# JuliaReinforcementLearning/ReinforcementLearning.jl

Hardware: AMD Instinct MI355X
Metric: env_steps_per_sec (higher is better)
Workload: dtype f32; 1 GPU; ppo_cartpole_4096env_per_gpu (BASELINE.json configs[3] per GPU); n_envs_per_gpu=4096, rollout_T=32, actor=4->256->2 relu, critic=4->256->1 relu, n_params=3331, n_epochs=4, n_microbatches=4, microbatch=32768, parallelism=single GPU

## Files before the change

### __graft_entry__.py

```python
import os
import sys

ROOT = os.path.dirname(os.path.abspath(__file__))
PKG = os.path.join(ROOT, "reinforcementlearning.jl_amd")
for p in (ROOT, PKG):
    if p not in sys.path:
        sys.path.insert(0, p)


def build():
    import importlib.util

    spec = importlib.util.spec_from_file_location("rlhip_build", os.path.join(PKG, "build.py"))
    mod = importlib.util.module_from_spec(spec)
    spec.loader.exec_module(mod)
    so = mod.build()
    assert os.path.exists(so)
    assert os.path.exists(mod.build(variant="bounds"))
    import oracle

    oracle.build()
    import rlhip

    missing = [s for s in rlhip._lib.declared_symbols() if not hasattr(rlhip._lib.lib, s)]
    assert not missing, f"librlhip.so does not export: {missing}"
    build_abi_host()
    build_micro_checks()


MICRO_CHECKS = ("mfma_f32_l1", "mfma_f32_4x4", "tanh_sel", "mfma_valu_overlap", "wave_simd_map", "log_sampling", "trig_f32arg")
MICRO_FLAGS = {"mfma_valu_overlap": ["-fno-slp-vectorize", "-fno-vectorize"], "trig_f32arg": ["-pthread"]}


def build_micro_checks():
    import subprocess

    outs = []
    for name in MICRO_CHECKS:
        src = os.path.join(ROOT, "tools", "micro", name + ".hip")
        out = os.path.join(ROOT, "tools", "micro", name + ".bin")
        if os.path.exists(out) and os.path.getmtime(out) >= max(
                [os.path.getmtime(src)] + [os.path.getmtime(os.path.join(PKG, "csrc", f)) for f in os.listdir(os.path.join(PKG, "csrc"))
                                           if f.endswith(".h")]):
            outs.append(out)
            continue
        cmd = ["/opt/rocm/bin/hipcc", "--offload-arch=gfx950", "-O3", "-std=c++17", "-ffp-contract=off", "-Wno-unused-result", "-Wno-unused-value",
               "-I" + os.path.join(ROOT, "include")] + MICRO_FLAGS.get(name, []) + [src, "-o", out]
        r = subprocess.run(cmd, capture_output=True, text=True)
        if r.returncode != 0:
            raise RuntimeError(f"hipcc failed for {src}:\n{r.stdout}\n{r.stderr}")
        outs.append(out)
    return outs


def build_abi_host():
    import subprocess

    src = os.path.join(ROOT, "tests", "abi_host", "abi_host.c")
    out = os.path.join(ROOT, "tests", "abi_host", "abi_host.bin")
    cmd = ["gcc", "-std=c99", "-O2", "-Wall", "-I" + os.path.join(ROOT, "include"), src, "-o", out,
           "-L" + os.path.join(PKG, "lib"), "-lrlhip", "-Wl,-rpath,$ORIGIN/../../reinforcementlearning.jl_amd/lib",
           "-Wl,-rpath,/opt/rocm/lib", "-lm"]
    r = subprocess.run(cmd, capture_output=True, text=True)
    if r.returncode != 0:
        raise RuntimeError(f"gcc failed for abi_host.c:\n{r.stdout}\n{r.stderr}")
    return out


def smoke():
    import numpy as np
    import torch

    import oracle
    import rlhip

    assert torch.cuda.is_available(), "smoke() needs an MI355X"
    torch.cuda.set_device(0)
    n, T = 256, 8
    env = rlhip.HipVecEnv("cartpole", n, seed=7)
    pol = rlhip.PPOPolicy(env, update_freq=T, n_epochs=1, n_microbatches=2)
    p0 = pol.params.cpu().numpy().copy()
    pol.rollout_()
    pol.gae_()
    tr = pol.trajectory
    oenv = oracle.VecEnv("cartpole", n, seed=7)
    ocfg = oracle.ppo_default(n_epochs=1, n_microbatches=2)
    otr = oracle.PPOTraj(0, n, T)
    oracle.ppo_rollout(oenv, T, ocfg, p0, otr, 0)
    agree = (tr.action_i.cpu().numpy() == otr.action_i).mean()
    assert agree > 0.995, f"sampled actions agree only {agree:.4f}"
    if agree == 1.0:
        assert np.array_equal(tr.terminal.cpu().numpy(), otr.terminal)
        np.testing.assert_allclose(tr.obs.cpu().numpy(), otr.obs, rtol=1e-5, atol=1e-6)
        np.testing.assert_allclose(tr.value.cpu().numpy(), otr.value, rtol=1e-5, atol=1e-6)
    o = oracle.generalized_advantage_estimation(tr.reward.cpu().numpy().T, tr.value.cpu().numpy().T, 0.99, 0.95,
                                                terminal=tr.terminal.cpu().numpy().T, dims=2, dtype=np.float32)
    assert np.array_equal(tr.adv.cpu().numpy(), o.T)
    pol.grad_(0, 0)
    total, bm = n * T, (n * T) // 2
    perm = np.array([oracle.permute(pol.seed, 0, total, b) for b in range(bm)])
    t, i = perm // n, perm % n
    obs = tr.obs.cpu().numpy()[t, :, i].T.copy()
    flat = lambda x: x.cpu().numpy().reshape(-1)[perm]
    g, losses = oracle.ppo_loss_grad(ocfg, 4, 2, p0, obs, flat(tr.action_i), flat(tr.logp), flat(tr.adv), flat(tr.ret))
    gerr = np.abs(pol.grad.cpu().numpy() - g).max() / np.abs(g).max()
    assert gerr <= 1e-6, f"gradient differs from the oracle by {gerr:.2e} of max|g| (bar 1e-6; measured 8e-8)"
    np.testing.assert_allclose(pol.losses.cpu().numpy(), losses, rtol=1e-4, atol=1e-6)
    pol.update_()
    torch.cuda.synchronize()
    assert torch.isfinite(pol.params).all() and not torch.equal(pol.params.cpu(), torch.tensor(p0))
    print(f"smoke ok: {n} envs x {T} steps, loss {float(pol.losses[0]):.5f}, actions agree {agree:.4f}")
    smoke_bench_shape(np, torch, oracle, rlhip)


def smoke_bench_shape(np, torch, oracle, rlhip):
    n, T = 4096, 32
    oracle.use_all_cores(True)
    try:
        env = rlhip.HipVecEnv("cartpole", n, seed=123)
        pol = rlhip.PPOPolicy(env, update_freq=T, hidden=256, seed=123)
        p0 = pol.params.cpu().numpy().copy()
        pol.rollout_()
        tr = pol.trajectory
        oenv = oracle.VecEnv("cartpole", n, seed=123)
        ocfg = oracle.ppo_default(hidden=256)
        otr = oracle.PPOTraj(0, n, T)
        oracle.ppo_rollout(oenv, T, ocfg, p0, otr, 0)
        ga = tr.action_i.cpu().numpy()
        flipped = (ga != otr.action_i).any(0)
        assert flipped.sum() <= 8, f"{flipped.sum()} of {n} envs took another action than the oracle's"
        keep = ~flipped
        assert np.array_equal(tr.terminal.cpu().numpy()[:, keep], otr.terminal[:, keep])
        np.testing.assert_allclose(tr.obs.cpu().numpy()[:, :, keep], otr.obs[:, :, keep], rtol=1e-5, atol=1e-6)
        np.testing.assert_allclose(tr.value.cpu().numpy()[:, keep], otr.value[:, keep], rtol=1e-5, atol=1e-6)
        mb, total = 1, n * T
        bm = total // pol.cfg.n_microbatches
        pol.grad_(0, mb)
        perm = np.array([oracle.permute(pol.seed, 0, total, mb * bm + b) for b in range(bm)])
        t, i = perm // n, perm % n
        flat = lambda x: x.cpu().numpy().reshape(-1)[perm]
        g, losses = oracle.ppo_loss_grad(ocfg, 4, 2, p0, tr.obs.cpu().numpy()[t, :, i].T.copy(), flat(tr.action_i), flat(tr.logp),
                                         flat(tr.adv), flat(tr.ret))
        gerr = np.abs(pol.grad.cpu().numpy() - g).max() / np.abs(g).max()
        assert bm == 32768 and gerr <= 1e-6, f"32768-sample gradient differs from the oracle by {gerr:.2e} of max|g| (bar 1e-6)"
        np.testing.assert_allclose(pol.losses.cpu().numpy(), losses, rtol=1e-4, atol=1e-6)
        print(f"smoke ok at the bench shape: {n} envs x {T} steps ({int(flipped.sum())} envs flipped an action), micro-batch of "
              f"{bm}: gradient within {gerr:.1e} of max|g|")
    finally:
        oracle.use_all_cores(False)


if __name__ == "__main__":
    build()
    if len(sys.argv) > 1 and sys.argv[1] == "smoke":
        smoke()
```

### reinforcementlearning.jl_amd/csrc/ppo.hip

```cpp
#include "env_device.h"
#include "mlp_device.h"
#include "select_device.h"
#include "select_decide.h"
#include "ppo_common.h"
#include "ppo_sample_device.h"

extern "C" int32_t rlhip_clip_adam_f32(float* params, float* grad, float* m, float* v, float* beta_pow,
                                       int64_t n, float grad_scale, float clip_norm, float lr, float beta1,
                                       float beta2, float eps, float* gn_out, rlhip_stream_t stream);
extern "C" int32_t rlhip_gae_returns_f32(float* advantages, float* returns, const float* rewards,
                                         const float* values, const uint8_t* terminal, int64_t n_env,
                                         int64_t T, float gamma, float lambda, rlhip_stream_t stream);

namespace rlhip {

__global__ void counters_advance_kernel(uint32_t* ctr, uint32_t d0, uint32_t d1) {
    ctr[0] += d0;
    ctr[1] += d1;
}

#ifdef RLHIP_ROLLOUT_TIMING
__device__ unsigned int g_rollout_exact_waves = 0;
#define RT_COUNT_EXACT()                                                   \
    do {                                                                   \
        if ((threadIdx.x & 63) == 0) atomicAdd(&g_rollout_exact_waves, 1u); \
    } while (0)
#define RT_PRINT_EXACT()                                                                                              \
    do {                                                                                                              \
        if (blockIdx.x == 0 && threadIdx.x == 0)                                                                      \
            printf("exact-selection wavefronts so far: %u\n", atomicAdd(&g_rollout_exact_waves, 0u));                  \
    } while (0)
#define RT_DECL long long rt_[8] = {0, 0, 0, 0, 0, 0, 0, 0}, rt_last_ = 0
#define RT_START() rt_last_ = (long long)__builtin_amdgcn_s_memtime()
#define RT_STAMP(k)                                                   \
    do {                                                              \
        __builtin_amdgcn_sched_barrier(0);                            \
        const long long now_ = (long long)__builtin_amdgcn_s_memtime(); \
        rt_[k] += now_ - rt_last_;                                    \
        rt_last_ = now_;                                              \
        __builtin_amdgcn_sched_barrier(0);                            \
    } while (0)
#define RT_PRINT(tag)                                                                                             \
    do {                                                                                                          \
        if (blockIdx.x == 0 && (threadIdx.x & 255) == 0)                                                          \
            printf("%s T=%d: %lld %lld %lld %lld %lld %lld %lld %lld\n", tag, T, rt_[0], rt_[1], rt_[2], rt_[3], rt_[4], \
                   rt_[5], rt_[6], rt_[7]);                                                                       \
    } while (0)
#else
#define RT_COUNT_EXACT()
#define RT_PRINT_EXACT()
#define RT_DECL
#define RT_START()
#define RT_STAMP(k)
#define RT_PRINT(tag)
#endif

template <class P, int H, int L, int ACT, int NOA, int HEAD>
__global__ __launch_bounds__(512, 1) void rollout_split_kernel(P p, EnvArrays<float> st, int64_t n, int T,
                                                               PolicyDesc pd, const float* __restrict__ params,
                                                               uint64_t seed, uint32_t env_id_base,
                                                               uint32_t vec_step0_in, const uint32_t* __restrict__ ctr, TrajPtrs tr,
                                                               int store_state, float select_margin) {
    const uint32_t vec_step0 = vec_step0_in + (ctr ? ctr[0] : 0u);
    constexpr int NS = P::ODIM;
    constexpr int HPL = H / L;
    constexpr int EPB = 256 / L;
    constexpr int NOISE_CH = 16;
    const int cont = HEAD == 0 ? pd.cont : (HEAD == 1 ? 1 : 0);
    const int na = HEAD == 0 ? pd.na : (HEAD == 1 ? 1 : HEAD);
    if (HEAD != 0) p.continuous = cont;
    const int role = (int)(threadIdx.x >> 8);
    const int tl = (int)(threadIdx.x & 255);
    int64_t gl = (int64_t)blockIdx.x * 256 + tl;
    int64_t env = gl / L;
    const int sub = (int)(gl % L);
    const int eg = tl / L;
    const bool active = env < n;
    if (!active) env = n - 1;
    const bool writer = active && sub == 0;
    const uint32_t id = env_id_base + (uint32_t)env;

    __shared__ double l_noise[2][EPB][NOISE_CH][MAXO];
    __shared__ float4 l_step[2][EPB][2];
    __shared__ float2 l_lse[HEAD == 2 ? EPB : 1][NOISE_CH];

    if (role == 0) {
        __builtin_amdgcn_s_setprio(3);
        NetRegs<NS, HPL> A;
        load_net<NS, HPL>(A, params, H, pd.nout_a, sub, L);
        LaneState<float> e;
#pragma unroll
        for (int k = 0; k < P::SDIM; ++k) e.s[k] = st.s[k][env];
        e.t = st.t[env];
        e.episode = st.episode[env];
        float last_r = 0.0f;
        bool last_d = false;
        [[maybe_unused]] const double sel_km = decide2_slope((double)select_margin);
        RT_DECL;
        __syncthreads();
        RT_START();
        for (int t = 0; t < T; ++t) {
            double nz[MAXO];
#pragma unroll
            for (int k = 0; k < MAXO; ++k)
                nz[k] = (HEAD == 2 ? k >= 2 : k < na) ? l_noise[(t / NOISE_CH) & 1][eg][t & (NOISE_CH - 1)][k] : 0.0;
            float x[4] = {0.f, 0.f, 0.f, 0.f};
            env_obs1(p, e, x);
            RT_STAMP(0);
            float oa[MAXO];
            net_forward<NS, HPL, L, ACT, NOA>(A, x, oa);
            RT_STAMP(1);
            int32_t ai;
            float af, lp;
            float sel_d = 0.0f;
            if constexpr (HEAD == 2) {
                float sel_e;
                bool decided;
                ai = decide2_logits(oa[0], oa[1], nz[2], nz[3], sel_km, &sel_e, &decided);
                decide2_operands(oa[0], oa[1], sel_e, ai, &lp, &sel_d);
                if (__builtin_amdgcn_ballot_w64(!decided) != 0) {
                    RT_COUNT_EXACT();
                    const double nzx[MAXO] = {l_noise[(t / NOISE_CH) & 1][eg][t & (NOISE_CH - 1)][0],
                                              l_noise[(t / NOISE_CH) & 1][eg][t & (NOISE_CH - 1)][1], 0.0, 0.0};
                    float lp_exact, xa0, xa1;
                    const int32_t ax = categorical_select1(RegLogits{oa}, NoMask{}, na, NoiseRegs{nzx}, &lp_exact);
                    if (!decided) ai = ax;
                    select2_operands(oa[0], oa[1], &xa0, &xa1, &sel_d);
                    lp = ai ? xa1 : xa0;
                }
                af = 0.0f;
            } else {
                policy_select(cont, na, oa, nz, ai, af, lp);
            }
            RT_STAMP(2);
            env_step1(p, e, ai, af, last_r, last_d);
            if (last_d) env_reset1(p, e, seed, id);
            RT_STAMP(3);
            if (sub == 0) {
                l_step[t & 1][eg][0] = make_float4(x[0], x[1], x[2], x[3]);
                if constexpr (HEAD == 2)
                    l_step[t & 1][eg][1] = make_float4(lp, sel_d, __int_as_float(ai | (last_d ? 0x100 : 0)), last_r);
                else
                    l_step[t & 1][eg][1] = make_float4(lp, cont ? af : __int_as_float(ai), last_r, last_d ? 1.0f : 0.0f);
            }
            RT_STAMP(4);
            __syncthreads();
            RT_STAMP(5);
        }
        RT_PRINT("actor wave: obs/noise | forward | select | env step | record | barrier");
        if (HEAD == 2) RT_PRINT_EXACT();
        {
            float x[4] = {0.f, 0.f, 0.f, 0.f};
            env_obs1(p, e, x);
            if (sub == 0) l_step[T & 1][eg][0] = make_float4(x[0], x[1], x[2], x[3]);
            __syncthreads();
        }
        if (writer && store_state) {
#pragma unroll
            for (int k = 0; k < P::SDIM; ++k) st.s[k][env] = e.s[k];
            st.t[env] = e.t;
            st.episode[env] = e.episode;
            if (T > 0) {
                st.reward[env] = last_r;
                st.done[env] = (uint8_t)last_d;
            }
        }
    } else {
        NetRegs<NS, HPL> C;
        load_net<NS, HPL>(C, params + pd.np_a, H, 1, sub, L);
        auto fill_noise = [&](int c0) {
            for (int i = sub; i < NOISE_CH && c0 + i < T; i += L) {
                double nz[MAXO] = {0.0, 0.0, 0.0, 0.0};
                policy_noise(cont, na, seed, id, vec_step0 + (uint32_t)(c0 + i), nz);
                if constexpr (HEAD == 2) decide2_noise_terms(nz[0], nz[1], (double)select_margin, &nz[2], &nz[3]);
#pragma unroll
                for (int k = 0; k < MAXO; ++k) l_noise[(c0 / NOISE_CH) & 1][eg][i][k] = nz[k];
            }
        };
        fill_noise(0);
        RT_DECL;
        __syncthreads();
        RT_START();
        for (int t = 0; t < T; ++t) {
            if ((t & (NOISE_CH - 1)) == 0 && t + NOISE_CH < T) fill_noise(t + NOISE_CH);
            RT_STAMP(0);
            __syncthreads();
            RT_STAMP(1);
            const float4 xv = l_step[t & 1][eg][0];
            const float x[4] = {xv.x, xv.y, xv.z, xv.w};
            float oc[MAXO];
            net_forward<NS, HPL, L, ACT, 1>(C, x, oc);
            RT_STAMP(2);
            if constexpr (HEAD == 2) {
                const float4 rec = l_step[t & 1][eg][1];
                if (sub == 0) l_lse[eg][t & (NOISE_CH - 1)] = make_float2(rec.x, rec.y);
                if (writer) {
#pragma unroll
                    for (int k = 0; k < NS; ++k) tr.obs[((int64_t)t * NS + k) * n + env] = x[k];
                    tr.value[(int64_t)t * n + env] = oc[0];
                    const int aw = __float_as_int(rec.z);
                    tr.action_i[(int64_t)t * n + env] = aw & 0xFF;
                    tr.reward[(int64_t)t * n + env] = rec.w;
                    tr.terminal[(int64_t)t * n + env] = (uint8_t)(aw >> 8);
                }
                if ((t & (L - 1)) == L - 1 || t + 1 == T) {
                    __builtin_amdgcn_fence(__ATOMIC_ACQ_REL, "wavefront");
                    __builtin_amdgcn_wave_barrier();
                    const int ts = (t & ~(L - 1)) + sub;
                    const float2 ad = l_lse[eg][ts & (NOISE_CH - 1)];
                    const float se = 1.0f + (float)::exp((double)ad.y);
                    const float lse = (float)log_f64_sampling((double)se);
                    if (active && ts <= t) tr.logp[(int64_t)ts * n + env] = ad.x - lse;
                    __builtin_amdgcn_fence(__ATOMIC_ACQ_REL, "wavefront");
                    __builtin_amdgcn_wave_barrier();
                }
            } else if (writer) {
                const float4 rec = l_step[t & 1][eg][1];
#pragma unroll
                for (int k = 0; k < NS; ++k) tr.obs[((int64_t)t * NS + k) * n + env] = x[k];
                tr.value[(int64_t)t * n + env] = oc[0];
                tr.logp[(int64_t)t * n + env] = rec.x;
                if (cont) tr.action_f[(int64_t)t * n + env] = rec.y;
                else tr.action_i[(int64_t)t * n + env] = __float_as_int(rec.y);
                tr.reward[(int64_t)t * n + env] = rec.z;
                tr.terminal[(int64_t)t * n + env] = (uint8_t)(rec.w != 0.0f);
            }
            RT_STAMP(3);
        }
        RT_PRINT("critic wave: noise | barrier | forward | stores");
        __syncthreads();
        {
            const float4 xv = l_step[T & 1][eg][0];
            const float x[4] = {xv.x, xv.y, xv.z, xv.w};
            float oc[MAXO];
            net_forward<NS, HPL, L, ACT, 1>(C, x, oc);
            if (writer) {
#pragma unroll
                for (int k = 0; k < NS; ++k) tr.obs[((int64_t)T * NS + k) * n + env] = x[k];
                tr.value[(int64_t)T * n + env] = oc[0];
            }
        }
        if (writer && T > 0 && tr.adv && tr.ret)
            gae_scan_lane(tr.adv, tr.ret, tr.reward, tr.value, tr.terminal, n, T, env, pd.gamma, pd.lambda);
    }
}

template <class P, int ACT>
__global__ __launch_bounds__(256) void rollout_scalar_kernel(P p, EnvArrays<float> st, int64_t n, int T,
                                                             PolicyDesc pd, const float* __restrict__ params,
                                                             uint64_t seed, uint32_t env_id_base,
                                                             uint32_t vec_step0_in, const uint32_t* __restrict__ ctr, TrajPtrs tr,
                                                              int store_state) {
    const uint32_t vec_step0 = vec_step0_in + (ctr ? ctr[0] : 0u);
    constexpr int NS = P::ODIM;
    int64_t env = (int64_t)blockIdx.x * blockDim.x + threadIdx.x;
    if (env >= n) return;
    uint32_t id = env_id_base + (uint32_t)env;
    LaneState<float> e;
#pragma unroll
    for (int k = 0; k < P::SDIM; ++k) e.s[k] = st.s[k][env];
    e.t = st.t[env];
    e.episode = st.episode[env];
    float last_r = 0.0f;
    bool last_d = false;
    for (int t = 0; t < T; ++t) {
        float x[4];
        env_obs1(p, e, x);
        float oa[MAXO], oc[MAXO];
        net_forward_scalar<NS, ACT>(params, pd.h, pd.nout_a, x, oa);
        net_forward_scalar<NS, ACT>(params + pd.np_a, pd.h, 1, x, oc);
        int32_t ai;
        float af, lp;
        policy_sample(pd.cont, pd.na, oa, seed, id, vec_step0 + (uint32_t)t, ai, af, lp);
#pragma unroll
        for (int k = 0; k < NS; ++k) tr.obs[((int64_t)t * NS + k) * n + env] = x[k];
        tr.value[(int64_t)t * n + env] = oc[0];
        tr.logp[(int64_t)t * n + env] = lp;
        if (pd.cont) tr.action_f[(int64_t)t * n + env] = af;
        else tr.action_i[(int64_t)t * n + env] = ai;
        env_step1(p, e, ai, af, last_r, last_d);
        if (last_d) env_reset1(p, e, seed, id);
        tr.reward[(int64_t)t * n + env] = last_r;
        tr.terminal[(int64_t)t * n + env] = (uint8_t)last_d;
    }
    {
        float x[4], oc[MAXO];
        env_obs1(p, e, x);
        net_forward_scalar<NS, ACT>(params + pd.np_a, pd.h, 1, x, oc);
#pragma unroll
        for (int k = 0; k < NS; ++k) tr.obs[((int64_t)T * NS + k) * n + env] = x[k];
        tr.value[(int64_t)T * n + env] = oc[0];
    }
    if (T > 0 && tr.adv && tr.ret)
        gae_scan_lane(tr.adv, tr.ret, tr.reward, tr.value, tr.terminal, n, T, env, pd.gamma, pd.lambda);
    if (store_state) {
#pragma unroll
        for (int k = 0; k < P::SDIM; ++k) st.s[k][env] = e.s[k];
        st.t[env] = e.t;
        st.episode[env] = e.episode;
        if (T > 0) {
            st.reward[env] = last_r;
            st.done[env] = (uint8_t)last_d;
        }
    }
}


template <class P>
static int32_t rollout_impl(const typename P::cfg_t* cfg, const rlhip_env_state* st, int64_t n, int64_t T,
                            const PolicyDesc& pd, const float* params, uint64_t seed, uint32_t env_id_base,
                            uint32_t vec_step0, const uint32_t* ctr, const rlhip_ppo_traj* traj, hipStream_t s) {
    RLHIP_REQUIRE(st && st->episode, "this entry point needs the separate episode[] array (packed step / episode words are an rlhip_env_step / rlhip_env_reset mode)");
    typename P::cfg_t c2 = *cfg;
    c2.continuous = pd.cont;
    P p = P::make(c2);
    EnvArrays<float> a = EnvArrays<float>::from(*st);
    TrajPtrs tr = TrajPtrs::from(*traj);
    static const float select_margin = []() {
        const char* e = getenv("RLHIP_ROLLOUT_SELECT_MARGIN");
        return (e && e[0]) ? strtof(e, nullptr) : 1.0f;
    }();
    RLHIP_REQUIRE(select_margin >= 1.0f, "RLHIP_ROLLOUT_SELECT_MARGIN must be a number >= 1 (or inf)");
    bool wide = (pd.h == 256 || pd.h == 128 || pd.h == 64) && n * 16 <= (int64_t)1 << 22;
#define LAUNCH_WIDE_AS(H, L, ACT_, NOA_, HEAD_)                                                                  \
    hipLaunchKernelGGL((rollout_split_kernel<P, H, L, ACT_, NOA_, HEAD_>), dim3((int)((n * L + 255) / 256)), dim3(512), \
                       0, s, p, a, n, (int)T, pd, params, seed, env_id_base, vec_step0, ctr, tr, 1, select_margin)
#define LAUNCH_WIDE(H, L)                                                                     \
    do {                                                                                      \
        if (pd.act == 0 && !pd.cont && pd.na == 2) LAUNCH_WIDE_AS(H, L, 0, 2, 2);             \
        else if (pd.act == 0 && pd.cont && pd.na == 1) LAUNCH_WIDE_AS(H, L, 0, 2, 1);         \
        else if (pd.act == 0 && !pd.cont && pd.na == 3) LAUNCH_WIDE_AS(H, L, 0, MAXO, 3);     \
        else if (pd.act == 0) LAUNCH_WIDE_AS(H, L, 0, MAXO, 0);                               \
        else if (!pd.cont && pd.na == 2) LAUNCH_WIDE_AS(H, L, 1, 2, 2);                       \
        else if (pd.cont && pd.na == 1) LAUNCH_WIDE_AS(H, L, 1, 2, 1);                        \
        else LAUNCH_WIDE_AS(H, L, 1, MAXO, 0);                                                \
    } while (0)
    if (wide && pd.h == 256) LAUNCH_WIDE(256, 16);
    else if (wide && pd.h == 128) LAUNCH_WIDE(128, 8);
    else if (wide && pd.h == 64) LAUNCH_WIDE(64, 4);
    else if (pd.act == 0)
        hipLaunchKernelGGL((rollout_scalar_kernel<P, 0>), dim3((int)((n + 255) / 256)), dim3(256), 0, s, p, a, n,
                           (int)T, pd, params, seed, env_id_base, vec_step0, ctr, tr, 1);
    else
        hipLaunchKernelGGL((rollout_scalar_kernel<P, 1>), dim3((int)((n + 255) / 256)), dim3(256), 0, s, p, a, n,
                           (int)T, pd, params, seed, env_id_base, vec_step0, ctr, tr, 1);
#undef LAUNCH_WIDE_AS
#undef LAUNCH_WIDE
    RLHIP_LAUNCH_CHECK();
    return RLHIP_OK;
}

template <int NS, int H, int L, int ACT>
__global__ __launch_bounds__(256, 1) void plan_wide_kernel(int64_t n, PolicyDesc pd,
                                                           const float* __restrict__ params,
                                                           const float* __restrict__ obs, uint64_t seed,
                                                           uint32_t env_id_base, uint32_t step,
                                                           int32_t* __restrict__ action_i,
                                                           float* __restrict__ action_f,
                                                           float* __restrict__ logp, float* __restrict__ value) {
    constexpr int HPL = H / L;
    int64_t gl = (int64_t)blockIdx.x * blockDim.x + threadIdx.x;
    int64_t env = gl / L;
    int sub = (int)(gl % L);
    bool active = env < n;
    if (!active) env = n - 1;
    NetRegs<NS, HPL> A, C;
    load_net<NS, HPL>(A, params, H, pd.nout_a, sub, L);
    load_net<NS, HPL>(C, params + pd.np_a, H, 1, sub, L);
    float x[NS];
#pragma unroll
    for (int k = 0; k < NS; ++k) x[k] = obs[(int64_t)k * n + env];
    float oa[MAXO], oc[MAXO];
    net_forward<NS, HPL, L, ACT>(A, x, oa);
    net_forward<NS, HPL, L, ACT>(C, x, oc);
    int32_t ai;
    float af, lp;
    policy_sample(pd.cont, pd.na, oa, seed, env_id_base + (uint32_t)env, step, ai, af, lp);
    if (active && sub == 0) {
        if (pd.cont) action_f[env] = af;
        else action_i[env] = ai;
        if (logp) logp[env] = lp;
        if (value) value[env] = oc[0];
    }
}

template <int NS, int ACT>
__global__ __launch_bounds__(256) void plan_scalar_kernel(int64_t n, PolicyDesc pd,
                                                          const float* __restrict__ params,
                                                          const float* __restrict__ obs, uint64_t seed,
                                                          uint32_t env_id_base, uint32_t step,
                                                          int32_t* __restrict__ action_i,
                                                          float* __restrict__ action_f, float* __restrict__ logp,
                                                          float* __restrict__ value) {
    int64_t env = (int64_t)blockIdx.x * blockDim.x + threadIdx.x;
    if (env >= n) return;
    float x[NS];
#pragma unroll
    for (int k = 0; k < NS; ++k) x[k] = obs[(int64_t)k * n + env];
    float oa[MAXO], oc[MAXO];
    net_forward_scalar<NS, ACT>(params, pd.h, pd.nout_a, x, oa);
    net_forward_scalar<NS, ACT>(params + pd.np_a, pd.h, 1, x, oc);
    int32_t ai;
    float af, lp;
    policy_sample(pd.cont, pd.na, oa, seed, env_id_base + (uint32_t)env, step, ai, af, lp);
    if (pd.cont) action_f[env] = af;
    else action_i[env] = ai;
    if (logp) logp[env] = lp;
    if (value) value[env] = oc[0];
}

template <int NS>
static int32_t plan_impl(int64_t n, const PolicyDesc& pd, const float* params, const float* obs, uint64_t seed,
                         uint32_t env_id_base, uint32_t step, int32_t* ai, float* af, float* logp, float* value,
                         hipStream_t s) {
    bool wide = (pd.h == 256 || pd.h == 128 || pd.h == 64) && n * 16 <= (int64_t)1 << 22;
#define LAUNCH_PW(H, L)                                                                                        \
    do {                                                                                                       \
        if (pd.act == 0)                                                                                       \
            hipLaunchKernelGGL((plan_wide_kernel<NS, H, L, 0>), dim3((int)((n * L + 255) / 256)), dim3(256), 0, s, n, \
                               pd, params, obs, seed, env_id_base, step, ai, af, logp, value);                \
        else                                                                                                   \
            hipLaunchKernelGGL((plan_wide_kernel<NS, H, L, 1>), dim3((int)((n * L + 255) / 256)), dim3(256), 0, s, n, \
                               pd, params, obs, seed, env_id_base, step, ai, af, logp, value);                \
    } while (0)
    if (wide && pd.h == 256) LAUNCH_PW(256, 16);
    else if (wide && pd.h == 128) LAUNCH_PW(128, 8);
    else if (wide && pd.h == 64) LAUNCH_PW(64, 4);
    else if (pd.act == 0)
        hipLaunchKernelGGL((plan_scalar_kernel<NS, 0>), dim3((int)((n + 255) / 256)), dim3(256), 0, s, n, pd, params,
                           obs, seed, env_id_base, step, ai, af, logp, value);
    else
        hipLaunchKernelGGL((plan_scalar_kernel<NS, 1>), dim3((int)((n + 255) / 256)), dim3(256), 0, s, n, pd, params,
                           obs, seed, env_id_base, step, ai, af, logp, value);
#undef LAUNCH_PW
    RLHIP_LAUNCH_CHECK();
    return RLHIP_OK;
}

__global__ __launch_bounds__(256) void mlp2_forward_kernel(const float* __restrict__ p, int n_in, int h,
                                                           int n_out, int act, const float* __restrict__ x,
                                                           int64_t batch, float* __restrict__ out) {
    int64_t i = (int64_t)blockIdx.x * blockDim.x + threadIdx.x;
    if (i >= batch) return;
    const float* W1 = p;
    const float* b1 = W1 + h * n_in;
    const float* W2 = b1 + h;
    const float* b2 = W2 + n_out * h;
    float xin[16], acc[32];
    for (int k = 0; k < n_in; ++k) xin[k] = x[(int64_t)k * batch + i];
    for (int o = 0; o < n_out; ++o) acc[o] = b2[o];
    for (int j = 0; j < h; ++j) {
        float z = b1[j];
        for (int k = 0; k < n_in; ++k) z = fmaf(W1[j + h * k], xin[k], z);
        float hv = act_fwd(act, z);
        for (int o = 0; o < n_out; ++o) acc[o] = fmaf(W2[o + n_out * j], hv, acc[o]);
    }
    for (int o = 0; o < n_out; ++o) out[(int64_t)o * batch + i] = acc[o];
}

__global__ __launch_bounds__(256) void mlp2_init_kernel(float* __restrict__ p, int n_in, int h, int n_out,
                                                        uint64_t seed, uint32_t net_id) {
    int64_t np = mlp2_nparams(n_in, h, n_out);
    int64_t q = (int64_t)blockIdx.x * blockDim.x + threadIdx.x;
    if (q >= np) return;
    int64_t o1 = (int64_t)h * n_in, o2 = o1 + h, o3 = o2 + (int64_t)n_out * h;
    float val = 0.0f;
    if (q < o1) {
        float s1 = sqrtf(6.0f / (float)(n_in + h));
        u32x4 w = philox4x32_10(seed, (uint32_t)q, 0, net_id * 4u + 0u, TAG_INIT);
        val = (2.0f * u01_f32(w.x) - 1.0f) * s1;
    } else if (q >= o2 && q < o3) {
        float s2 = sqrtf(6.0f / (float)(h + n_out));
        u32x4 w = philox4x32_10(seed, (uint32_t)(q - o2), 0, net_id * 4u + 2u, TAG_INIT);
        val = (2.0f * u01_f32(w.x) - 1.0f) * s2;
    }
    p[q] = val;
}

__global__ __launch_bounds__(256) void ppo_push_preact_kernel(TrajPtrs tr, int64_t t, int ns, int64_t n,
                                                              const float* __restrict__ obs, const float* __restrict__ value,
                                                              const float* __restrict__ logp,
                                                              const int32_t* __restrict__ a_i, const float* __restrict__ a_f) {
    for (int64_t i = (int64_t)blockIdx.x * blockDim.x + threadIdx.x; i < n; i += (int64_t)gridDim.x * blockDim.x) {
        for (int k = 0; k < ns; ++k) tr.obs[(t * ns + k) * n + i] = obs[(int64_t)k * n + i];
        tr.value[t * n + i] = value[i];
        if (logp) tr.logp[t * n + i] = logp[i];
        if (a_i) tr.action_i[t * n + i] = a_i[i];
        if (a_f) tr.action_f[t * n + i] = a_f[i];
    }
}
__global__ __launch_bounds__(256) void ppo_push_postact_kernel(TrajPtrs tr, int64_t t, int64_t n,
                                                               const float* __restrict__ reward,
                                                               const uint8_t* __restrict__ done) {
    for (int64_t i = (int64_t)blockIdx.x * blockDim.x + threadIdx.x; i < n; i += (int64_t)gridDim.x * blockDim.x) {
        tr.reward[t * n + i] = reward[i];
        tr.terminal[t * n + i] = done[i];
    }
}

}

using namespace rlhip;

extern "C" {

int32_t rlhip_ppo_default(rlhip_ppo_cfg* c) {
    RLHIP_REQUIRE(c != nullptr, "cfg is NULL");
    c->gamma = 0.99f;
    c->lambda = 0.95f;
    c->clip_range = 0.1f;
    c->max_grad_norm = 0.5f;
    c->actor_loss_weight = 1.0f;
    c->critic_loss_weight = 0.5f;
    c->entropy_loss_weight = 0.001f;
    c->lr = 1e-3f;
    c->beta1 = 0.9f;
    c->beta2 = 0.999f;
    c->adam_eps = 1e-8f;
    c->n_epochs = 4;
    c->n_microbatches = 4;
    c->hidden = 256;
    c->act = 0;
    c->continuous = 0;
    c->normalize_advantage = 0;
    c->layers = 2;
    return RLHIP_OK;
}

int64_t rlhip_ppo_nparams(int32_t kind, const rlhip_ppo_cfg* c) {
    if (is_layers3(c)) return ppo3_nparams(kind, c);
    PolicyDesc pd;
    if (make_desc(kind, c, &pd)) return -1;
    int ns = kind == 0 ? 4 : (kind == 1 ? 3 : 2);
    return pd.np_a + mlp2_nparams(ns, pd.h, 1);
}

int64_t rlhip_mlp2_nparams(int64_t n_in, int64_t h, int64_t n_out) { return mlp2_nparams(n_in, h, n_out); }

int32_t rlhip_mlp2_forward_f32(const float* params, int64_t n_in, int64_t h, int64_t n_out, int32_t act,
                               const float* x, int64_t batch, float* out, rlhip_stream_t stream) {
    RLHIP_REQUIRE(params && x && out, "NULL array");
    RLHIP_REQUIRE(n_in >= 1 && n_in <= 16 && n_out >= 1 && n_out <= 32 && h >= 1, "unsupported layer sizes");
    RLHIP_REQUIRE(act == 0 || act == 1, "act must be 0 (relu) or 1 (tanh)");
    if (batch == 0) return RLHIP_OK;
    hipLaunchKernelGGL(mlp2_forward_kernel, dim3((int)((batch + 255) / 256)), dim3(256), 0, as_stream(stream),
                       params, (int)n_in, (int)h, (int)n_out, act, x, batch, out);
    RLHIP_LAUNCH_CHECK();
    return RLHIP_OK;
}

int32_t rlhip_mlp2_init_f32(float* params, int64_t n_in, int64_t h, int64_t n_out, uint64_t seed,
                            uint32_t net_id, rlhip_stream_t stream) {
    RLHIP_REQUIRE(params != nullptr && n_in >= 1 && h >= 1 && n_out >= 1, "bad arguments");
    int64_t np = mlp2_nparams(n_in, h, n_out);
    hipLaunchKernelGGL(mlp2_init_kernel, dim3((int)((np + 255) / 256)), dim3(256), 0, as_stream(stream), params,
                       (int)n_in, (int)h, (int)n_out, seed, net_id);
    RLHIP_LAUNCH_CHECK();
    return RLHIP_OK;
}

int32_t rlhip_ppo_plan_f32(int32_t kind, const rlhip_ppo_cfg* cfg, const float* params, const float* obs,
                           int64_t n, uint64_t seed, uint32_t env_id_base, uint32_t vec_step,
                           int32_t* action_i, float* action_f, float* logp, float* value,
                           rlhip_stream_t stream) {
    RLHIP_REQUIRE(!is_layers3(cfg), "layers = 3: use the fused rollout (rlhip_ppo_rollout_f32), the per-step plan! is "
                                    "not built for the MFMA actor / critic");
    PolicyDesc pd;
    int32_t rc = make_desc(kind, cfg, &pd);
    if (rc) return rc;
    RLHIP_REQUIRE(params && obs && n >= 0, "bad arguments");
    RLHIP_REQUIRE(pd.cont ? (action_f != nullptr) : (action_i != nullptr), "action output is NULL");
    if (n == 0) return RLHIP_OK;
    hipStream_t s = as_stream(stream);
    if (kind == 0) return plan_impl<4>(n, pd, params, obs, seed, env_id_base, vec_step, action_i, action_f, logp, value, s);
    if (kind == 1) return plan_impl<3>(n, pd, params, obs, seed, env_id_base, vec_step, action_i, action_f, logp, value, s);
    return plan_impl<2>(n, pd, params, obs, seed, env_id_base, vec_step, action_i, action_f, logp, value, s);
}

int32_t rlhip_ppo_push_preact_f32(const rlhip_ppo_traj* traj, int64_t t, int64_t ns, int64_t n, const float* obs,
                                  const float* value, const float* logp, const int32_t* action_i, const float* action_f,
                                  rlhip_stream_t stream) {
    RLHIP_REQUIRE(traj && traj->obs && traj->value && obs && value, "NULL argument");
    RLHIP_REQUIRE(t >= 0 && ns >= 1 && ns <= 8 && n >= 0, "bad slot / shape");
    RLHIP_REQUIRE(!logp || traj->logp, "trajectory has no logp trace");
    RLHIP_REQUIRE((!action_i || traj->action_i) && (!action_f || traj->action_f), "trajectory has no action trace");
    if (n == 0) return RLHIP_OK;
    hipLaunchKernelGGL(ppo_push_preact_kernel, dim3(grid_for(n, 256)), dim3(256), 0, as_stream(stream), TrajPtrs::from(*traj),
                       t, (int)ns, n, obs, value, logp, action_i, action_f);
    RLHIP_LAUNCH_CHECK();
    return RLHIP_OK;
}

int32_t rlhip_ppo_push_postact_f32(const rlhip_ppo_traj* traj, int64_t t, int64_t n, const float* reward,
                                   const uint8_t* done, rlhip_stream_t stream) {
    RLHIP_REQUIRE(traj && traj->reward && traj->terminal && reward && done, "NULL argument");
    RLHIP_REQUIRE(t >= 0 && n >= 0, "bad slot / shape");
    if (n == 0) return RLHIP_OK;
    hipLaunchKernelGGL(ppo_push_postact_kernel, dim3(grid_for(n, 256)), dim3(256), 0, as_stream(stream),
                       TrajPtrs::from(*traj), t, n, reward, done);
    RLHIP_LAUNCH_CHECK();
    return RLHIP_OK;
}

static int32_t rollout_entry(int32_t kind, const void* env_cfg, const rlhip_env_state* st, int64_t n, int64_t T,
                             const rlhip_ppo_cfg* cfg, const float* params, uint64_t seed, uint32_t env_id_base,
                             uint32_t vec_step0, const uint32_t* ctr, const rlhip_ppo_traj* traj,
                             rlhip_stream_t stream) {
    RLHIP_REQUIRE(kind != 1 || !cfg || cfg->continuous || !env_cfg || ((const rlhip_pendulum_cfg*)env_cfg)->n_actions == 3,
                  "PPO on a discrete Pendulum needs n_actions = 3 (the policy head has 3 actions)");
    if (is_layers3(cfg)) {
        RLHIP_REQUIRE(ctr == nullptr, "layers = 3: the device-counter (graph replay) variant is not built");
        return ppo3_rollout(kind, env_cfg, st, n, T, cfg, params, seed, env_id_base, vec_step0, traj, stream);
    }
    PolicyDesc pd;
    int32_t rc = make_desc(kind, cfg, &pd);
    if (rc) return rc;
    RLHIP_REQUIRE(env_cfg && st && params && traj, "NULL argument");
    RLHIP_REQUIRE(n >= 1 && n <= 0x7FFFFFFFll && T >= 0 && T <= 0x7FFFFFFFll, "bad n / T");
    RLHIP_REQUIRE(traj->obs && traj->logp && traj->value && traj->reward && traj->terminal, "trajectory array is NULL");
    RLHIP_REQUIRE(pd.cont ? (traj->action_f != nullptr) : (traj->action_i != nullptr), "action trace is NULL");
    hipStream_t s = as_stream(stream);
    if (kind == 0)
        return rollout_impl<CartPoleParams<float>>((const rlhip_cartpole_cfg*)env_cfg, st, n, T, pd, params, seed, env_id_base, vec_step0, ctr, traj, s);
    if (kind == 1)
        return rollout_impl<PendulumParams<float>>((const rlhip_pendulum_cfg*)env_cfg, st, n, T, pd, params, seed, env_id_base, vec_step0, ctr, traj, s);
    return rollout_impl<MountainCarParams<float>>((const rlhip_mountaincar_cfg*)env_cfg, st, n, T, pd, params, seed, env_id_base, vec_step0, ctr, traj, s);
}

int32_t rlhip_ppo_rollout_f32(int32_t kind, const void* env_cfg, const rlhip_env_state* st, int64_t n,
                              int64_t T, const rlhip_ppo_cfg* cfg, const float* params, uint64_t seed,
                              uint32_t env_id_base, uint32_t vec_step0, const rlhip_ppo_traj* traj,
                              rlhip_stream_t stream) {
    return rollout_entry(kind, env_cfg, st, n, T, cfg, params, seed, env_id_base, vec_step0, nullptr, traj, stream);
}

int32_t rlhip_ppo_rollout_dc_f32(int32_t kind, const void* env_cfg, const rlhip_env_state* st, int64_t n,
                                 int64_t T, const rlhip_ppo_cfg* cfg, const float* params, uint64_t seed,
                                 uint32_t env_id_base, const uint32_t* counters, const rlhip_ppo_traj* traj,
                                 rlhip_stream_t stream) {
    RLHIP_REQUIRE(counters != nullptr, "counters is NULL");
    return rollout_entry(kind, env_cfg, st, n, T, cfg, params, seed, env_id_base, 0, counters, traj, stream);
}

int32_t rlhip_counters_advance(uint32_t* counters, uint32_t d_vec_step, uint32_t d_update, rlhip_stream_t stream) {
    RLHIP_REQUIRE(counters != nullptr, "counters is NULL");
    hipLaunchKernelGGL(counters_advance_kernel, dim3(1), dim3(1), 0, as_stream(stream), counters, d_vec_step, d_update);
    RLHIP_LAUNCH_CHECK();
    return RLHIP_OK;
}

int32_t rlhip_ppo_gae_f32(const rlhip_ppo_cfg* cfg, int64_t n, int64_t T, const rlhip_ppo_traj* traj,
                          rlhip_stream_t stream) {
    RLHIP_REQUIRE(cfg && traj && traj->adv && traj->ret && traj->reward && traj->value && traj->terminal,
                  "NULL argument");
    return rlhip_gae_returns_f32(traj->adv, traj->ret, traj->reward, traj->value, traj->terminal, n, T,
                                 cfg->gamma, cfg->lambda, stream);
}


}
```

Measured before the change: 357.4 million env-steps/s.

## Replace per-step actor/critic block barrier with an 8-slot LDS ring handoff

```diff
diff --git a/__graft_entry__.py b/__graft_entry__.py
--- a/__graft_entry__.py
+++ b/__graft_entry__.py
@@ -17,6 +17,7 @@
     so = mod.build()
     assert os.path.exists(so)
     assert os.path.exists(mod.build(variant="bounds"))
+    assert os.path.exists(mod.build(variant="rollout_timing"))
     import oracle
 
     oracle.build()
diff --git a/reinforcementlearning.jl_amd/csrc/ppo.hip b/reinforcementlearning.jl_amd/csrc/ppo.hip
--- a/reinforcementlearning.jl_amd/csrc/ppo.hip
+++ b/reinforcementlearning.jl_amd/csrc/ppo.hip
@@ -1,7 +1,10 @@
+#include <string.h>
+
 #include "env_device.h"
 #include "mlp_device.h"
 #include "select_device.h"
 #include "select_decide.h"
+#include "rollout_ring.h"
 #include "ppo_common.h"
 #include "ppo_sample_device.h"
 
@@ -40,6 +43,7 @@
         rt_last_ = now_;                                              \
         __builtin_amdgcn_sched_barrier(0);                            \
     } while (0)
+#define RT_COUNT(k) rt_[k] += 1
 #define RT_PRINT(tag)                                                                                             \
     do {                                                                                                          \
         if (blockIdx.x == 0 && (threadIdx.x & 255) == 0)                                                          \
@@ -52,20 +56,35 @@
 #define RT_DECL
 #define RT_START()
 #define RT_STAMP(k)
+#define RT_COUNT(k)
 #define RT_PRINT(tag)
 #endif
 
-template <class P, int H, int L, int ACT, int NOA, int HEAD>
-__global__ __launch_bounds__(512, 1) void rollout_split_kernel(P p, EnvArrays<float> st, int64_t n, int T,
-                                                               PolicyDesc pd, const float* __restrict__ params,
-                                                               uint64_t seed, uint32_t env_id_base,
-                                                               uint32_t vec_step0_in, const uint32_t* __restrict__ ctr, TrajPtrs tr,
-                                                               int store_state, float select_margin) {
+constexpr int RING_SPIN_MAX = 1 << 18;
+
+__device__ __forceinline__ int ring_load(const int* w) {
+    return __builtin_amdgcn_readfirstlane(__hip_atomic_load(w, __ATOMIC_RELAXED, __HIP_MEMORY_SCOPE_WORKGROUP));
+}
+__device__ __forceinline__ void ring_store(int* w, int v) {
+    __builtin_amdgcn_fence(__ATOMIC_RELEASE, "wavefront");
+    if ((threadIdx.x & 63) == 0) __hip_atomic_store(w, v, __ATOMIC_RELAXED, __HIP_MEMORY_SCOPE_WORKGROUP);
+}
+__device__ __forceinline__ void rollout_stall(int rounds) {
+    for (int i = 0; i < rounds; ++i) __builtin_amdgcn_s_sleep(4);
+}
+
+template <class P, int H, int L, int ACT, int NOA, int HEAD, bool RING>
+__device__ __forceinline__ void rollout_two_wave(P p, EnvArrays<float> st, int64_t n, int T, PolicyDesc pd,
+                                                 const float* __restrict__ params, uint64_t seed, uint32_t env_id_base,
+                                                 uint32_t vec_step0_in, const uint32_t* __restrict__ ctr, TrajPtrs tr,
+                                                 int store_state, float select_margin, int stall) {
     const uint32_t vec_step0 = vec_step0_in + (ctr ? ctr[0] : 0u);
     constexpr int NS = P::ODIM;
     constexpr int HPL = H / L;
     constexpr int EPB = 256 / L;
     constexpr int NOISE_CH = 16;
+    using Ring = RolloutRing<ROLLOUT_RING_R>;
+    constexpr int NSLOT = RING ? ROLLOUT_RING_R : 2;
     const int cont = HEAD == 0 ? pd.cont : (HEAD == 1 ? 1 : 0);
     const int na = HEAD == 0 ? pd.na : (HEAD == 1 ? 1 : HEAD);
     if (HEAD != 0) p.continuous = cont;
@@ -81,8 +100,12 @@
     const uint32_t id = env_id_base + (uint32_t)env;
 
     __shared__ double l_noise[2][EPB][NOISE_CH][MAXO];
-    __shared__ float4 l_step[2][EPB][2];
+    __shared__ float4 l_step[NSLOT][EPB][2];
     __shared__ float2 l_lse[HEAD == 2 ? EPB : 1][NOISE_CH];
+    __shared__ int l_flag[RING ? 4 : 1][2];
+    [[maybe_unused]] int* const l_pub = &l_flag[RING ? (threadIdx.x >> 6) & 3 : 0][0];
+    [[maybe_unused]] int* const l_done = l_pub + 1;
+    auto slot = [](int t) { return RING ? Ring::slot(t) : (t & 1); };
 
     if (role == 0) {
         __builtin_amdgcn_s_setprio(3);
@@ -97,6 +120,21 @@
         bool last_d = false;
         [[maybe_unused]] const double sel_km = decide2_slope((double)select_margin);
         RT_DECL;
+        [[maybe_unused]] auto wait_slot = [&](int t, int dn) {
+            if (!Ring::actor_may_write(t, dn)) {
+                RT_COUNT(6);
+                __builtin_amdgcn_s_setprio(0);
+                int rounds = 0;
+                do {
+                    __builtin_amdgcn_s_sleep(1);
+                    RT_COUNT(7);
+                    dn = ring_load(l_done);
+                } while (!Ring::actor_may_write(t, dn) && ++rounds < RING_SPIN_MAX);
+                __builtin_amdgcn_s_setprio(3);
+            }
+            __builtin_amdgcn_fence(__ATOMIC_ACQUIRE, "workgroup");
+        };
+        if (RING && threadIdx.x < 8) (&l_flag[0][0])[threadIdx.x] = 0;
         __syncthreads();
         RT_START();
         for (int t = 0; t < T; ++t) {
@@ -104,6 +142,8 @@
 #pragma unroll
             for (int k = 0; k < MAXO; ++k)
                 nz[k] = (HEAD == 2 ? k >= 2 : k < na) ? l_noise[(t / NOISE_CH) & 1][eg][t & (NOISE_CH - 1)][k] : 0.0;
+            [[maybe_unused]] int dn = 0;
+            if constexpr (RING) dn = ring_load(l_done);
             float x[4] = {0.f, 0.f, 0.f, 0.f};
             env_obs1(p, e, x);
             RT_STAMP(0);
@@ -135,25 +175,30 @@
             RT_STAMP(2);
             env_step1(p, e, ai, af, last_r, last_d);
             if (last_d) env_reset1(p, e, seed, id);
+            if (stall < 0) rollout_stall(-stall);
             RT_STAMP(3);
+            if constexpr (RING) wait_slot(t, dn);
             if (sub == 0) {
-                l_step[t & 1][eg][0] = make_float4(x[0], x[1], x[2], x[3]);
+                l_step[slot(t)][eg][0] = make_float4(x[0], x[1], x[2], x[3]);
                 if constexpr (HEAD == 2)
-                    l_step[t & 1][eg][1] = make_float4(lp, sel_d, __int_as_float(ai | (last_d ? 0x100 : 0)), last_r);
+                    l_step[slot(t)][eg][1] = make_float4(lp, sel_d, __int_as_float(ai | (last_d ? 0x100 : 0)), last_r);
                 else
-                    l_step[t & 1][eg][1] = make_float4(lp, cont ? af : __int_as_float(ai), last_r, last_d ? 1.0f : 0.0f);
+                    l_step[slot(t)][eg][1] = make_float4(lp, cont ? af : __int_as_float(ai), last_r, last_d ? 1.0f : 0.0f);
             }
             RT_STAMP(4);
-            __syncthreads();
+            if constexpr (RING) ring_store(l_pub, Ring::published(t));
+            else __syncthreads();
             RT_STAMP(5);
         }
-        RT_PRINT("actor wave: obs/noise | forward | select | env step | record | barrier");
+        RT_PRINT("actor wave: obs/noise | forward | select | env step | record (+ slot wait) | hand-over | slot waits | wait rounds");
         if (HEAD == 2) RT_PRINT_EXACT();
         {
             float x[4] = {0.f, 0.f, 0.f, 0.f};
             env_obs1(p, e, x);
-            if (sub == 0) l_step[T & 1][eg][0] = make_float4(x[0], x[1], x[2], x[3]);
-            __syncthreads();
+            if constexpr (RING) wait_slot(T, ring_load(l_done));
+            if (sub == 0) l_step[slot(T)][eg][0] = make_float4(x[0], x[1], x[2], x[3]);
+            if constexpr (RING) ring_store(l_pub, Ring::published(T));
+            else __syncthreads();
         }
         if (writer && store_state) {
 #pragma unroll
@@ -177,22 +222,30 @@
                 for (int k = 0; k < MAXO; ++k) l_noise[(c0 / NOISE_CH) & 1][eg][i][k] = nz[k];
             }
         };
+        [[maybe_unused]] auto wait_record = [&](int t) {
+            int rounds = 0;
+            while (!Ring::critic_may_read(t, ring_load(l_pub)) && ++rounds < RING_SPIN_MAX) __builtin_amdgcn_s_sleep(1);
+            __builtin_amdgcn_fence(__ATOMIC_ACQUIRE, "workgroup");
+        };
         fill_noise(0);
         RT_DECL;
         __syncthreads();
         RT_START();
         for (int t = 0; t < T; ++t) {
             if ((t & (NOISE_CH - 1)) == 0 && t + NOISE_CH < T) fill_noise(t + NOISE_CH);
+            if (stall > 0) rollout_stall(stall);
             RT_STAMP(0);
-            __syncthreads();
+            if constexpr (RING) wait_record(t);
+            else __syncthreads();
             RT_STAMP(1);
-            const float4 xv = l_step[t & 1][eg][0];
+            const float4 xv = l_step[slot(t)][eg][0];
+            const float4 rec = l_step[slot(t)][eg][1];
+            if constexpr (RING) ring_store(l_done, Ring::consumed(t));
             const float x[4] = {xv.x, xv.y, xv.z, xv.w};
             float oc[MAXO];
             net_forward<NS, HPL, L, ACT, 1>(C, x, oc);
             RT_STAMP(2);
             if constexpr (HEAD == 2) {
-                const float4 rec = l_step[t & 1][eg][1];
                 if (sub == 0) l_lse[eg][t & (NOISE_CH - 1)] = make_float2(rec.x, rec.y);
                 if (writer) {
 #pragma unroll
@@ -215,7 +268,6 @@
                     __builtin_amdgcn_wave_barrier();
                 }
             } else if (writer) {
-                const float4 rec = l_step[t & 1][eg][1];
 #pragma unroll
                 for (int k = 0; k < NS; ++k) tr.obs[((int64_t)t * NS + k) * n + env] = x[k];
                 tr.value[(int64_t)t * n + env] = oc[0];
@@ -227,10 +279,11 @@
             }
             RT_STAMP(3);
         }
-        RT_PRINT("critic wave: noise | barrier | forward | stores");
-        __syncthreads();
+        RT_PRINT("critic wave: noise | barrier / poll | forward | stores");
+        if constexpr (RING) wait_record(T);
+        else __syncthreads();
         {
-            const float4 xv = l_step[T & 1][eg][0];
+            const float4 xv = l_step[slot(T)][eg][0];
             const float x[4] = {xv.x, xv.y, xv.z, xv.w};
             float oc[MAXO];
             net_forward<NS, HPL, L, ACT, 1>(C, x, oc);
@@ -243,6 +296,26 @@
         if (writer && T > 0 && tr.adv && tr.ret)
             gae_scan_lane(tr.adv, tr.ret, tr.reward, tr.value, tr.terminal, n, T, env, pd.gamma, pd.lambda);
     }
+}
+
+template <class P, int H, int L, int ACT, int NOA, int HEAD>
+__global__ __launch_bounds__(512, 1) void rollout_split_kernel(P p, EnvArrays<float> st, int64_t n, int T,
+                                                               PolicyDesc pd, const float* __restrict__ params,
+                                                               uint64_t seed, uint32_t env_id_base,
+                                                               uint32_t vec_step0_in, const uint32_t* __restrict__ ctr, TrajPtrs tr,
+                                                               int store_state, float select_margin, int stall) {
+    rollout_two_wave<P, H, L, ACT, NOA, HEAD, false>(p, st, n, T, pd, params, seed, env_id_base, vec_step0_in, ctr, tr, store_state,
+                                                     select_margin, stall);
+}
+
+template <class P, int H, int L, int ACT, int NOA, int HEAD>
+__global__ __launch_bounds__(512, 1) void rollout_ring_kernel(P p, EnvArrays<float> st, int64_t n, int T,
+                                                              PolicyDesc pd, const float* __restrict__ params,
+                                                              uint64_t seed, uint32_t env_id_base,
+                                                              uint32_t vec_step0_in, const uint32_t* __restrict__ ctr, TrajPtrs tr,
+                                                              int store_state, float select_margin, int stall) {
+    rollout_two_wave<P, H, L, ACT, NOA, HEAD, true>(p, st, n, T, pd, params, seed, env_id_base, vec_step0_in, ctr, tr, store_state,
+                                                    select_margin, stall);
 }
 
 template <class P, int ACT>
@@ -321,10 +394,35 @@
         return (e && e[0]) ? strtof(e, nullptr) : 1.0f;
     }();
     RLHIP_REQUIRE(select_margin >= 1.0f, "RLHIP_ROLLOUT_SELECT_MARGIN must be a number >= 1 (or inf)");
+    static const int handover_barrier = []() {
+        const char* e = getenv("RLHIP_ROLLOUT_HANDOVER");
+        if (!e || !e[0] || !strcmp(e, "ring")) return 0;
+        return !strcmp(e, "barrier") ? 1 : -1;
+    }();
+    RLHIP_REQUIRE(handover_barrier >= 0, "RLHIP_ROLLOUT_HANDOVER must be `ring` or `barrier`");
+    static const int stall = []() {
+        const char* e = getenv("RLHIP_ROLLOUT_STALL");
+        if (!e || !e[0]) return 0;
+        const bool critic = !strncmp(e, "critic:", 7), actor = !strncmp(e, "actor:", 6);
+        if (!critic && !actor) return INT32_MIN;
+        char* end = nullptr;
+        const long k = strtol(e + (critic ? 7 : 6), &end, 10);
+        if (end == e + (critic ? 7 : 6) || *end || k < 0 || k > 100000) return INT32_MIN;
+        return critic ? (int)k : -(int)k;
+    }();
+    RLHIP_REQUIRE(stall != INT32_MIN, "RLHIP_ROLLOUT_STALL must be critic:K or actor:K with 0 <= K <= 100000");
     bool wide = (pd.h == 256 || pd.h == 128 || pd.h == 64) && n * 16 <= (int64_t)1 << 22;
-#define LAUNCH_WIDE_AS(H, L, ACT_, NOA_, HEAD_)                                                                  \
-    hipLaunchKernelGGL((rollout_split_kernel<P, H, L, ACT_, NOA_, HEAD_>), dim3((int)((n * L + 255) / 256)), dim3(512), \
-                       0, s, p, a, n, (int)T, pd, params, seed, env_id_base, vec_step0, ctr, tr, 1, select_margin)
+#define LAUNCH_WIDE_AS(H, L, ACT_, NOA_, HEAD_)                                                                         \
+    do {                                                                                                                \
+        if (handover_barrier)                                                                                           \
+            hipLaunchKernelGGL((rollout_split_kernel<P, H, L, ACT_, NOA_, HEAD_>), dim3((int)((n * L + 255) / 256)),    \
+                               dim3(512), 0, s, p, a, n, (int)T, pd, params, seed, env_id_base, vec_step0, ctr, tr, 1,  \
+                               select_margin, stall);                                                                   \
+        else                                                                                                            \
+            hipLaunchKernelGGL((rollout_ring_kernel<P, H, L, ACT_, NOA_, HEAD_>), dim3((int)((n * L + 255) / 256)),     \
+                               dim3(512), 0, s, p, a, n, (int)T, pd, params, seed, env_id_base, vec_step0, ctr, tr, 1,  \
+                               select_margin, stall);                                                                   \
+    } while (0)
 #define LAUNCH_WIDE(H, L)                                                                     \
     do {                                                                                      \
         if (pd.act == 0 && !pd.cont && pd.na == 2) LAUNCH_WIDE_AS(H, L, 0, 2, 2);             \
diff --git a/reinforcementlearning.jl_amd/csrc/rollout_ring.h b/reinforcementlearning.jl_amd/csrc/rollout_ring.h
--- /dev/null
+++ b/reinforcementlearning.jl_amd/csrc/rollout_ring.h
@@ -0,0 +1,24 @@
+#pragma once
+#include <stdint.h>
+
+#if defined(__HIPCC__) || defined(__CUDACC__)
+#define RLHIP_RING_HD __host__ __device__
+#else
+#define RLHIP_RING_HD
+#endif
+
+namespace rlhip {
+
+constexpr int ROLLOUT_RING_R = 8;
+
+template <int R>
+struct RolloutRing {
+    static_assert(R >= 4 && R <= 8 && (R & (R - 1)) == 0, "R: a power of two, 4 <= R <= 8");
+    RLHIP_RING_HD static int slot(int t) { return t & (R - 1); }
+    RLHIP_RING_HD static bool actor_may_write(int t, int done) { return done >= t + 1 - R; }
+    RLHIP_RING_HD static bool critic_may_read(int t, int pub) { return pub >= t + 1; }
+    RLHIP_RING_HD static int published(int t) { return t + 1; }
+    RLHIP_RING_HD static int consumed(int t) { return t + 1; }
+};
+
+}
```

Result: no change. 356.6 million env-steps/s (-0.2%).
